# zblz/naima

Hardware: AMD Instinct MI355X
Metric: walker-steps/sec (ensemble lnprob evals/s) (higher is better)
Workload: dtype f64

## Files before the change

### naima_amd/csrc/nh_halfstep.hip

```cpp
#include "nh_hs_plan.h"
#include <memory>

typedef int hs_i16 __attribute__((ext_vector_type(16)));
typedef int hs_i8 __attribute__((ext_vector_type(8)));
typedef int hs_i2 __attribute__((ext_vector_type(2)));
typedef int hs_i4 __attribute__((ext_vector_type(4)));
template <class T>
__device__ __forceinline__ const T __attribute__((address_space(1))) * hs_gptr(int lo, int hi) {
  return (const T __attribute__((address_space(1)))*)(((unsigned long long)(unsigned)hi << 32) |
                                                      (unsigned)lo);
}
#define HS_KERNARG_H 48
static_assert(offsetof(hs_hot, F) == 0, "hs_first leads the argument block");
static_assert(sizeof(hs_hot) + HS_KERNARG_H <= 0xcc0, "the warm-up loads cover the argument block");
static_assert(sizeof(hs_hot) + HS_KERNARG_H >= 0xc84, "the last warm-up load (0xc80) stays inside the argument block");
static_assert(sizeof(hs_first) == 256 && offsetof(hs_first, qT) == 224 &&
                  offsetof(hs_first, syn_c) == 240 && offsetof(hs_first, nG) == 48 &&
                  offsetof(hs_first, e) == 64 && offsetof(hs_first, lne) == 128 &&
                  offsetof(hs_first, pkd) == 192, "hs_first: the layout the first trip reads");
__device__ __attribute__((noinline)) double hs_log_ool(double x) { return log(x); }
template <bool SYN, bool S2 = false>
__global__ __launch_bounds__(1024) void k_half_step(const int* __restrict__ done_,
                                                    const double* __restrict__ blk_,
                                                    const double* coords_, int slice, int ns_,
// ... 975 lines not shown
}

extern "C" int nh_table_interleave(nh_ctx* c, const double* Kt, const double* dlnKt,
                                   const double* lx, int nG, int nK, double* KD) {
  NH_REQUIRE(c && Kt && dlnKt && KD && nG >= 0 && nK >= 0, "bad argument");
  const long long n = (long long)nG * nK;
  if (n == 0) return NH_OK;
  nh_prof_scope ps(c, NH_K_TABLES);
  hipLaunchKernelGGL(k_table_interleave, dim3((unsigned)((n + 255) / 256)), dim3(256), 0, c->stream,
                     Kt, dlnKt, lx, nG, nK, KD);
  NH_CHECK_HIP(hipGetLastError());
  return NH_OK;
}

__global__ void k_syn_consts(const double* __restrict__ gam, const double* __restrict__ lx, int nG,
                             double* __restrict__ out) {
  const int i = blockIdx.x * blockDim.x + threadIdx.x;
  if (i >= nG) return;
  const double gi = gam[i];
  const double v = 1.0 / (gi * gi);
  out[i] = v;
  out[nG + i] = cbrt(v);
  out[2 * nG + i] = i + 1 < nG ? v * expm1(-2.0 * lx[i]) : 0.0;
}

__global__ void k_set_word(int* p, int v) { *p = v; }
__global__ void k_set_word2(int* p, int v0, int v1) {
  p[0] = v0;
  p[1] = v1;
}

__global__ void k_hist_append(const double* __restrict__ coords, const double* __restrict__ logp,
                              long long N, int ndim, const nh_hist* hist, long long row) {
  if (row < 0) row = hist->n - 1;
  if (!hist->coords || row < 0 || row >= hist->cap) return;
  const long long nc = N * ndim;
  double* hc = hist->coords + row * nc;
  double* hl = hist->logp + row * N;
  for (long long t = threadIdx.x; t < nc; t += blockDim.x) hc[t] = coords[t];
  for (long long t = threadIdx.x; t < N; t += blockDim.x) hl[t] = logp[t];
}

extern "C" int nh_hist_append(nh_ctx* c, const double* coords, const double* logp, long long N,
                              int ndim, const nh_hist* hist, long long row) {
  NH_REQUIRE(c && coords && logp && hist && N >= 1 && ndim >= 1, "bad argument");
  nh_prof_scope ps(c, NH_K_GLUE);
  hipLaunchKernelGGL(k_hist_append, dim3(1), dim3(1024), 0, c->stream, coords, logp, N, ndim, hist,
                     row);
  NH_CHECK_HIP(hipGetLastError());
  return NH_OK;
}

static hs_opt hs_env_opt(const char* name) {
  const char* e = getenv(name);
  hs_opt o;
  o.set = e != nullptr;
  o.v = e ? atoi(e) : 0;
  return o;
}
hs_knobs hs_knobs_read() {
  hs_knobs k = hs_knobs_default();
  k.test_reject = getenv("NH_HS_TEST_REJECT") != nullptr;
  if (const char* e = getenv("NH_HS_SPLIT")) k.kmax = atoi(e) > 0 ? atoi(e) : 1;
  k.part_kb = nh_env_int("NH_HS_PART_KB", k.part_kb);
  k.threads = hs_env_opt("NH_HS_THREADS");
  k.split_min_work = nh_env_int("NH_HS_SPLIT_MIN_WORK", k.split_min_work);
  k.rowsplit = nh_env_int("NH_HS_ROWSPLIT", k.rowsplit);
  k.rt = nh_env_int("NH_HS_RT", k.rt);
  k.syn2 = nh_env_int("NH_HS_SYN2", k.syn2);
  k.rt_debug = getenv("NH_HS_RT_DEBUG") != nullptr;
  k.seg = hs_env_opt("NH_HS_SEG");
  k.syn_nodes = hs_env_opt("NH_HS_SYN_NODES");
  k.debug = nh_env_int("NH_HS_DEBUG", 0) != 0;
  k.run_rt = nh_env_int("NH_RUN_RT", k.run_rt);
  k.run_grids_in_lds = nh_env_int("NH_RUN_GRIDS_IN_LDS", k.run_grids_in_lds);
  k.run_ut = nh_env_int("NH_RUN_UT", k.run_ut);
  k.run_rowsplit = nh_env_int("NH_RUN_ROWSPLIT", k.run_rowsplit);
  k.run_syn2 = nh_env_int("NH_RUN_SYN2", k.run_syn2);
  k.run_il = nh_env_int("NH_RUN_IL", k.run_il);
  k.run_rebalance = hs_env_opt("NH_RUN_REBALANCE");
  k.run_tcompact_min = nh_env_int("NH_RUN_TCOMPACT_MIN", k.run_tcompact_min);
  k.run_syn_nodes = hs_env_opt("NH_RUN_SYN_NODES");
  k.run_pipeline = nh_env_int("NH_RUN_PIPELINE", k.run_pipeline);
  k.run_fail_at = nh_env_int("NH_RUN_FAIL_AT", 0);
  k.run_grid = hs_env_opt("NH_RUN_GRID");
  k.run_max_per_wg = hs_env_opt("NH_RUN_MAX_PER_WG");
  k.run_shared_alloc = nh_env_int("NH_RUN_SHARED_ALLOC", k.run_shared_alloc);
  k.run_spin_limit = hs_env_opt("NH_RUN_SPIN_LIMIT");
  k.run_publish_delay = nh_env_int("NH_RUN_PUBLISH_DELAY", 0);
  return k;
}

bool hs_read_grid(const double* xg, int nG, std::vector<double>& out) {
  out.assign((size_t)nG, 0.0);
  if (hipMemcpy(out.data(), xg, (size_t)nG * sizeof(double), hipMemcpyDeviceToHost) == hipSuccess) return true;
  (void)hipGetLastError();
  return false;
}

static void hs_gather(nh_ctx* c, const nh_hs_desc* d, const hs_knobs& k, hs_facts& f, std::vector<double>& xg) {
  f.ncu = nh_cu_count(256);
  f.syn_xg = nullptr;
  for (int t = 0; t < HS_MAX_TAB; ++t) f.r0[t] = -1;
  if (d->ngrids < 1 || d->ngrids > NH_MAX_GRIDS) return;
  const bool want_xg = d->syn.grid >= 0 && d->syn.grid < d->ngrids && k.syn2 != 0 &&
                       d->grids[d->syn.grid].xg && d->grids[d->syn.grid].nG >= 2;
  const bool want_rows = hs_plan_reads_rows(d, k, f.ncu);
  if ((!want_xg && !want_rows) || nh_sync(c) != NH_OK) return;
  if (want_xg && hs_read_grid(d->grids[d->syn.grid].xg, d->grids[d->syn.grid].nG, xg)) f.syn_xg = xg.data();
  for (int t = 0; t < d->ntab && want_rows; ++t) {
    const nh_hs_table& tb = d->tab[t];
    if (tb.grid < 0 || tb.grid >= d->ngrids || !tb.KD || tb.nK < 1 || d->grids[tb.grid].nG < 2) break;
    const int nG = d->grids[tb.grid].nG, nK = tb.nK;
    if ((size_t)nG * nK * 16 > ((size_t)64 << 20)) break;
    std::vector<double> kd((size_t)nG * nK * 2);
    if (hipMemcpy(kd.data(), tb.KD, kd.size() * sizeof(double), hipMemcpyDeviceToHost) != hipSuccess) {
      (void)hipGetLastError();
      break;
    }
    int r0 = nG - 1;
    for (int i = 0; i < nG - 1 && r0 == nG - 1; ++i)
      for (int q = 0; q < nK; ++q)
        if (kd[((size_t)i * nK + q) * 2] != 0.0) { r0 = i; break; }
    f.r0[t] = r0;
  }
}

static int hs_create(nh_ctx* c, const nh_hs_desc* d, nh_halfstep_plan** out) {
  NH_REQUIRE(c && d && out, "NULL pointer");
  const hs_knobs k = hs_knobs_read();
  hs_facts facts;
  std::vector<double> xg;
  hs_gather(c, d, k, facts, xg);
  std::unique_ptr<nh_halfstep_plan> P(new nh_halfstep_plan());
  hs_hot& H = P->hot;
  hs_shape S;
  const int rc = hs_plan(d, k, facts, H, S);
  if (rc != NH_OK) return rc;
  P->span = 3;
  P->lds_bytes = S.lds_bytes;
  P->lds_core = S.lds_core;
  P->threads = S.threads;
  P->blocks = d->nloc;
  P->split = S.split;
  P->rowsplit = S.rowsplit ? 1 : 0;
  P->rt = S.rt ? 1 : 0;
  nh_owned& m = P->mem;
  const int nspec = H.C.nspec;
  if (k.debug) {
    P->dbg = m.dev<long long>(67840 * sizeof(long long));
    m.fill(c, P->dbg, 0, 67840 * sizeof(long long));
  }
  P->dev = m.dev<nh_pack>(sizeof(S.packs));
  if (H.syn_grid >= 0) {
    const int nGs = H.nG[H.syn_grid];
    const size_t ns2 = H.o_s2 ? HS_S2_HDR + S.s2.data.size() : 0;
    P->syn_c = m.dev<double>((3 * (size_t)nGs + ns2) * sizeof(double));
    if (m.ok()) {
      hipLaunchKernelGGL(k_syn_consts, dim3((unsigned)((nGs + 255) / 256)), dim3(256), 0, c->stream,
                         H.xg[H.syn_grid], H.lx[H.syn_grid], nGs, P->syn_c);
      m.check(hipGetLastError());
    }
    if (m.ok() && ns2) {
      const hs_s2_host& s2h = S.s2;
      std::vector<double> up(ns2, 0.0);
      up[0] = s2h.par.ilx; up[1] = s2h.par.th; up[2] = s2h.par.im; up[3] = s2h.par.lml;
// ... 162 lines not shown
```

### naima_amd/csrc/nh_hs_plan.h

```cpp
#pragma once
#include "nh_hs.h"
#include "nh_syn2.h"

#define HS_RUN_MAX_STEPS 32
#define HS_RUN_ERR_TIMEOUT 1
#define HS_RUN_ERR_PEER 2
#define HS_RUN_ERR_LAST_ROW 3
#define HS_RUN_MAX_RANKS 8
#define HS_RUN_HEAD 512
#define HS_O_HX 56
enum { HX_PRE = 0, HX_SPECRD = 1 };
#define HS_O_LNA 48
#define HS_RUN_TRAIL 16
#define HS_RUN_PKW 8

enum { HSU_FL = 0, HSU_NL, HSU_G, HSU_W, HSU_D, HSU_DP, HSU_IL, HSU_TH, HSU_LX, HSU_LNE, HSU_GX, HSU_GE,
       HSU_S2LW, HSU_S2LG, HSU_SC_LO, HSU_SC_HI, HSU_N };
static_assert(HSU_N == 16, "a unit's descriptor is four 16-byte reads");

enum { HST_KD_LO = 0, HST_KD_HI, HST_NK, HST_NG, HST_AW, HST_AD, HST_AL, HST_FLAGS, HST_SUB, HST_NKP,
       HST_N = 16 };
#define HSI_N 4

struct hs_run {
  unsigned long long* ring;
  int* status;
  int* accw;
  double* hcoords; double* hlogp;
  double* hblob[NH_HS_MAX_BLOB];
  long long hrow0, hcap;
  long long* dbg;
  double* xspec; int* tick;
  int slice0, nslices;
  unsigned seq;
  int gr, N;
  int o_gx[NH_MAX_GRIDS], o_lne[NH_MAX_GRIDS], o_ge[NH_MAX_GRIDS];
  int o_pk, o_small1, o_olds;
  int o_lcl;
  int o_trail;
  const double* kds[HS_MAX_TAB];
  int spin_limit;
  int syn_nodes;
  int rebalance;
  int* report;
  int report_launch;
  int* lcnt;
  int o_il[NH_MAX_GRIDS];
  int o_ut;
  int o_it;
  int o_sum, o_cmp;
  int o_pci;
  int o_mt;
  int o_lnt;
  int o_synce;
  int rowsplit;
  int tcompact;
  int o_rs;
  int nxmax;
  int sum_cols;
  int nrank, rank;
  unsigned long long* peer[HS_RUN_MAX_RANKS];
  int* nacc_own;
  int* hacc;
  int* curstamp;
  int stamp0;
  int publish_delay;
  int syn2, s2_own;
  int o_s2tab, o_s2lw, o_s2ig, o_s2lg, o_s2q, o_s2z, o_s2t;
  const double* s2_dev;
  hs_syn2_par s2;
  double s2_z0, s2_invd;
  double s2_r746;
  double s2_lnw0;
  int pipeline;
  long long* clk;
};

static_assert(sizeof(hs_hot) + sizeof(hs_run) <= 4000, "both argument blocks fit the kernarg segment");

struct hs_opt {
  bool set;
  int v;
  int or_else(int dflt) const { return set ? v : dflt; }
};
struct hs_knobs {
  bool test_reject;
  int kmax;
  int part_kb;
  hs_opt threads;
  int split_min_work;
  int rowsplit, rt, syn2;
  bool rt_debug;
  hs_opt seg, syn_nodes;
  bool debug;
  int run_rt, run_grids_in_lds, run_ut, run_rowsplit, run_syn2, run_il;
  hs_opt run_rebalance;
  int run_tcompact_min;
  hs_opt run_syn_nodes;
  int run_pipeline;
  int run_fail_at;
  hs_opt run_grid;
  hs_opt run_max_per_wg;
  int run_shared_alloc;
  hs_opt run_spin_limit;
  int run_publish_delay;
};
static inline hs_knobs hs_knobs_default() {
  hs_knobs k;
  memset(&k, 0, sizeof(k));
  k.kmax = 8; k.part_kb = 40; k.split_min_work = 1 << 20;
  k.rowsplit = k.rt = k.syn2 = 1;
  k.run_rt = k.run_grids_in_lds = k.run_ut = k.run_rowsplit = k.run_syn2 = k.run_il = 1;
  k.run_tcompact_min = 4; k.run_pipeline = 1; k.run_shared_alloc = 1;
  return k;
}

struct hs_facts {
  int ncu;
  const double* syn_xg;
  int r0[HS_MAX_TAB];
};
static inline bool hs_plan_reads_rows(const nh_hs_desc* d, const hs_knobs& k, int ncu) {
  return d->syn.grid < 0 && d->ntab > 0 && d->ntab <= NH_HS_MAX_TAB && d->nloc <= ncu && k.rt != 0;
}

#define HSP_REQUIRE(cond, msg)                                               \
  do {                                                                       \
    if (!(cond)) return nh_set_error(NH_EINVAL, "%s: %s", who, msg);         \
  } while (0)
#define HS_S2_HDR 16

struct hs_shape {
  int threads, split, segscale;
  bool rowsplit, rt;
  size_t lds_core, lds_bytes;
  hs_s2_host s2;
  nh_pack packs[NH_MAX_PACK];
};
struct hs_plan_front {
  int off, nspec, syn_nE, threads;
  long long work;
  bool s2_ok;
};

static inline int hs_plan_checked(const nh_hs_desc* d, const hs_knobs& k, const hs_facts& f, hs_hot& H,
                                  hs_shape& S, hs_plan_front& A) {
  static const char* who = "hs_create";
  HSP_REQUIRE(d->coords && d->logp && d->blk && d->cursor && d->qT && d->factors && d->params &&
                  d->total, "NULL pointer in the descriptor");
  HSP_REQUIRE(d->ns >= 1 && d->ndim >= 1 && d->ndim <= 64 && d->lo >= 0 && d->nloc >= 1 &&
                  d->lo + d->nloc <= d->ns, "bad proposal block");
  HSP_REQUIRE(!d->do_accept || (d->lo == 0 && d->nloc == d->ns && d->accepted),
              "the in-kernel accept needs every walker of the slice in this launch");
  HSP_REQUIRE(d->npacks >= 1 && d->npacks <= NH_MAX_PACK, "bad pack plan");
  HSP_REQUIRE(d->kind >= NH_PD_POWERLAW && d->kind <= NH_PD_LOGPARABOLA, "unknown particle distribution kind");
  HSP_REQUIRE(d->ngrids >= 1 && d->ngrids <= NH_MAX_GRIDS, "bad grid count");
  HSP_REQUIRE(d->nmoms >= 0 && d->nmoms <= NH_MAX_MOMENT, "bad reductions");
  HSP_REQUIRE(d->ntab >= 0 && d->ntab <= NH_HS_MAX_TAB && (d->ntab > 0 || d->syn.grid >= 0),
              "a half-step needs at least one emission component");
  HSP_REQUIRE(d->ncomp >= 1 && d->ncomp <= NH_MAX_COMP && d->nE >= 1, "bad likelihood components");
  HSP_REQUIRE(d->conv && d->flux && d->err_lo && d->err_hi && d->ul && d->cl, "NULL data column");
  HSP_REQUIRE(d->nterms >= 0 && d->nterms <= NH_MAX_PRIOR, "bad prior terms");
  static_assert(NH_HS_MAX_TAB == HS_MAX_TAB, "table count");
  static_assert(sizeof(hs_hot) <= 3800, "the by-value kernel argument must fit the 4 KB segment");
  memset(&H, 0, sizeof(H));
  hs_dev& C = H.C;
  memset(S.packs, 0, sizeof(S.packs));
  H.coords = d->coords; H.logp = d->logp; H.blk = d->blk; H.cursor = d->cursor;
  H.qT = d->qT; H.factors = d->factors; H.hist = d->hist;
  H.ns = d->ns; H.ndim = d->ndim; H.lo = d->lo; H.nloc = d->nloc;
  C.npk = d->npacks; C.kind = d->kind; C.params = d->params;
  bool have_params = false;
  for (int q = 0; q < d->npacks; ++q) {
    const nh_pack& pk = d->packs[q];
    HSP_REQUIRE(pk.out && pk.ncols >= 1 && pk.ncols <= NH_MAX_LAZY && pk.ld >= pk.ncols,
                "bad pack request");
    for (int c = 0; c < pk.ncols; ++c) {
      const double* b = pk.cols[c].base;
      HSP_REQUIRE(b == nullptr || (b >= d->qT && b < d->qT + (long long)d->ndim * d->nloc &&
                                   (b - d->qT) % d->nloc == 0 && pk.cols[c].stride == 1),
                  "a pack column must read one proposal coordinate (or be a constant)");
    }
    if (pk.out == d->params) {
      HSP_REQUIRE(pk.ncols >= 7, "the particle rows need 7 columns");
      have_params = true;
    }
    S.packs[q] = pk;
  }
  HSP_REQUIRE(have_params, "params must be the output of one of the packs");
  HSP_REQUIRE(d->ndim < 255, "at most 254 fit parameters");
  for (int t = 0; t < d->ntab; ++t) {
    const nh_hs_table& tb = d->tab[t];
    HSP_REQUIRE(tb.grid >= 0 && tb.grid < d->ngrids && tb.KD && tb.out && tb.nK >= 1 &&
                    tb.ldo >= tb.nK, "bad table reduction");
  }
  if (k.test_reject)
// ... 304 lines not shown
  bool rt = P->rt != 0 && H.syn_grid < 0 && H.ntab > 0 && P->threads <= 512 && k.run_rt != 0;
  rt = rt && H.C.nT <= (P->threads / 64) * P->split;
  const bool grids_in_lds = (P->threads >= 1024 || rt) && k.run_grids_in_lds != 0;
  for (int g = 0; g < NH_MAX_GRIDS; ++g) R.o_gx[g] = R.o_lne[g] = R.o_ge[g] = -1;
  for (int g = 0; g < H.ngrids && grids_in_lds; ++g) {
    R.o_gx[g] = off; off += H.nG[g];
    R.o_lne[g] = off; off += H.nG[g];
    R.o_ge[g] = off;
    if (H.F.broken & 1) off += H.nG[g];
  }
  for (int g = 0; g < NH_MAX_GRIDS; ++g) R.o_il[g] = -1;
  R.rebalance = k.run_rebalance.or_else(H.syn_grid < 0 ? 1 : 0);
  const bool units_tab = grids_in_lds && k.run_ut != 0;
  R.rowsplit = (P->rowsplit && P->split >= 2 && units_tab && R.rebalance && H.ntab == 1 &&
                HS_CHUNKS(H.C.tab[0].chunks) % P->split == 0 && H.C.nT % P->split == 0 &&
                k.run_rowsplit != 0) ? 1 : 0;
  R.tcompact = P->split >= k.run_tcompact_min ? 1 : 0;
  int hole_lo = 0, hole_hi = 0;
  if (R.tcompact) {
    int nsmax = 0;
    if (H.syn_grid >= 0) nsmax = (H.syn_nE * H.C.syn_cdmax + 63) / 64;
    const int nslots = R.rowsplit ? H.C.nT / P->split : (H.C.nT + nsmax) / P->split + 2;
    if (nslots < H.C.nT) {
      hole_lo = H.o_part_t + nslots * 64;
      hole_hi = H.o_part_t + H.C.nT * 64;
    } else {
      R.tcompact = 0;
    }
  }
  auto take = [&](int n, bool align16) {
    if (align16) hole_lo += hole_lo & 1;
    if (hole_lo + n <= hole_hi) {
      const int at = hole_lo;
      hole_lo += n;
      return at;
    }
    if (align16) off += off & 1;
    const int at = off;
    off += n;
    return at;
  };
  R.o_ut = -1;
  if (units_tab) {
    int nunits = 0;
    for (int g = 0; g < H.ngrids; ++g) nunits += (H.nG[g] + 63) / 64;
    R.o_ut = take(nunits * (HSU_N / 2), true);
  }
  {
    int ncols = 0;
    for (int t = 0; t < H.ntab; ++t) ncols += H.C.tab[t].nK;
    R.sum_cols = ncols;
    R.o_sum = take(ncols, false);
    R.o_cmp = take(2 * NH_MAX_COMP + 2, false);
    R.o_pci = take((NH_MAX_PRIOR + 1) / 2, false);
    R.o_synce = H.syn_grid >= 0 ? take(H.syn_nE, false) : -1;
    R.o_lnt = -1;
    R.o_mt = take(4 * NH_MAX_MOMENT, true);
    {
      int nun = 0;
      for (int g = 0; g < H.ngrids; ++g) nun += (H.nG[g] + 63) / 64;
      R.o_rs = take((9 + nun + 2 * NH_MAX_GRIDS + 1) / 2, false);
    }
    R.nxmax = H.C.nspec + NH_MAX_MOMENT;
  }
  for (int t = 0; t < H.ntab; ++t)
    HSP_REQUIRE(H.nG[H.C.tab[t].grid] < 65536, "a table's grid has too many nodes for the items' descriptors");
  R.o_it = -1;
  if (!rt && H.C.nT > 0)
    R.o_it = take((HS_MAX_TAB * HST_N + H.C.nT * HSI_N + 1) / 2, true);
  R.o_pk = take(NH_MAX_PACK * NH_MAX_LAZY * HS_RUN_PKW, false);
  R.o_small1 = take(HS_O_T64, false);
  R.o_olds = take(128, false);
  R.o_lcl = take(H.nE + 1, false);
  R.o_trail = take((HS_RUN_TRAIL * HS_MAX_TAB + H.C.nspec + 1) / 2, false);
  for (int t = 0; t < H.ntab; ++t)
    HSP_REQUIRE(H.C.tab[t].tiles <= HS_RUN_TRAIL, "a table of more column tiles than the resident loop stages");
  R.syn2 = 0;
  R.s2_dev = nullptr;
  if (H.syn_grid >= 0 && k.run_syn2 != 0 && syn_xg != nullptr &&
      hs_s2_prepare(syn_xg, H.nG[H.syn_grid], H.scale[H.syn_grid], 8, S.s2)) {
    const int nG = H.nG[H.syn_grid], Pn = S.s2.par.P;
    R.s2 = S.s2.par;
    R.s2_invd = S.s2.invd; R.s2_lnw0 = S.s2.lnw0; R.s2_z0 = S.s2.z0; R.s2_r746 = S.s2.r746;
    const int off_was = off, hole_was = hole_lo;
    R.o_s2tab = take((Pn + 1) * HS_S2_STRIDE, true);
    const int sg = H.syn_grid;
    bool own = nG >= 2 * HS_S2_GUARD && H.o_d[sg] == H.o_w[sg] + nG && H.o_ig23 == H.o_dig2 + nG;
    for (int t = 0; t < H.ntab; ++t) own = own && H.C.tab[t].grid != sg;
    for (int q = 0; q < H.nmom; ++q) own = own && H.mgrid[q] != sg;
    R.s2_own = own ? 1 : 0;
    if (own) {
      R.o_s2lw = H.o_w[sg];
      R.o_s2ig = H.o_dig2;
    } else {
      R.o_s2lw = take(nG + 2 * HS_S2_GUARD, false);
      R.o_s2ig = take(nG + 2 * HS_S2_GUARD, false);
    }
    if (own && grids_in_lds) {
      R.o_s2lg = R.o_gx[sg];
    } else {
      R.o_s2lg = take(nG, false);
    }
    R.o_s2q = take(4 * H.syn_nE, false);
    R.o_s2z = take((H.syn_nE + 1) / 2, false);
    R.o_s2t = take(HS_S2_TN, false);
    R.o_lnt = take(256, true);
    if ((size_t)off * sizeof(double) <= 160 * 1024) {
      R.syn2 = 1;
    } else {
      off = off_was;
      hole_lo = hole_was;
    }
  }
  if (k.run_il != 0)
    for (int g = 0; g < H.ngrids; ++g)
      if (H.o_dp[g] >= 0 && (hole_lo + H.nG[g] <= hole_hi || (size_t)(off + H.nG[g]) * sizeof(double) <= 158 * 1024))
        R.o_il[g] = take(H.nG[g], false);
  R.syn_nodes = H.C.syn_nodes;
  if (P->split == 1 && R.syn_nodes < 32) R.syn_nodes = R.syn2 ? 48 : 32;
  if (P->split == 2 && R.syn_nodes < 10) R.syn_nodes = 10;
  if (R.syn2 && P->split >= 2 && R.syn_nodes < 16) R.syn_nodes = 16;
  R.syn_nodes = k.run_syn_nodes.or_else(R.syn_nodes);
  R.pipeline = k.run_pipeline;
  if (k.run_fail_at > 0)
    fprintf(stderr, "libnaima_hip: NH_RUN_FAIL_AT=%d -- that launch of the resident loop is made to time "
                    "out (fault injection of the tests)\n", k.run_fail_at);
  HSP_REQUIRE(R.syn_nodes >= 1, "NH_RUN_SYN_NODES must be positive");
  const size_t lds = (size_t)off * sizeof(double);
  HSP_REQUIRE(lds <= 160 * 1024, "the resident loop's working set does not fit in LDS");
  S.rt = rt;
  S.lds_bytes = lds;
  return NH_OK;
}

static inline int hs_run_grid(const nh_halfstep_plan* P, bool shared, bool rt, const hs_run& R, const hs_knobs& k,
                              int per_cu, int ncu, int* grid, bool* deep_candidate) {
  static const char* who = "hs_run_create";
  const hs_hot& H = P->hot;
  HSP_REQUIRE(per_cu >= 1 && ncu >= 1, "the resident kernel does not fit a compute unit");
  long long cap = (long long)per_cu * ncu;
  if (k.run_grid.set) cap = k.run_grid.v > 0 ? k.run_grid.v : cap;
  const long long per_wg = k.run_max_per_wg.or_else(P->threads >= 1024 ? 8 : 1);
  HSP_REQUIRE((long long)H.nloc * P->split <= cap * (per_wg > 1 ? per_wg : 1),
              "more walkers per half-step than resident workgroups");
  *grid = (int)(H.nloc < cap / P->split ? H.nloc : cap / P->split);
  *deep_candidate = !shared && !rt && H.syn_grid >= 0 && P->split == 1 && P->threads >= 1024 &&
                    H.nloc > *grid && R.pipeline != 0;
  return NH_OK;
}

hs_knobs hs_knobs_read();
bool hs_read_grid(const double* xg, int nG, std::vector<double>& out);
```

### naima_amd/csrc/nh_persist.hip

```cpp
#include "nh_hs_plan.h"
#include <memory>
#include <vector>
#include <chrono>
#include <unistd.h>

#ifndef HS_RUN_PK
#define HS_RUN_PK 5
#endif

__device__ __forceinline__ unsigned long long hs_ld_sc1(const unsigned long long* p) {
  return __hip_atomic_load(p, __ATOMIC_RELAXED, __HIP_MEMORY_SCOPE_AGENT);
}
__device__ __forceinline__ void hs_st_sc1(unsigned long long* p, unsigned long long v) {
  __hip_atomic_store(p, v, __ATOMIC_RELAXED, __HIP_MEMORY_SCOPE_AGENT);
}
__device__ __forceinline__ unsigned long long hs_ld_sys(const unsigned long long* p) {
  return __hip_atomic_load(p, __ATOMIC_RELAXED, __HIP_MEMORY_SCOPE_SYSTEM);
}
__device__ __forceinline__ void hs_st_sys(unsigned long long* p, unsigned long long v) {
  __hip_atomic_store(p, v, __ATOMIC_RELAXED, __HIP_MEMORY_SCOPE_SYSTEM);
}
__device__ __forceinline__ unsigned hs_tag(unsigned seq, int row) {
  return (seq << 8) | (unsigned)(row + 1);
}
// ... 243 lines not shown
#define HSR_STAMP(k)                                                                   \
  do {                                                                                  \
    if (R.dbg && tid == 0 && blockIdx.x < 256 && it < 64)                               \
      R.dbg[((long long)blockIdx.x * 64 + it) * 8 + (k)] = (long long)wall_clock64();   \
  } while (0)

struct hsr_a_out { double pval; int pcol, bad, ok; };
template <bool SYN, bool MULTI, bool S2, int RT = 0, bool DEEP = false>
__global__ __launch_bounds__(RT > 0 ? 512 : 1024) void k_half_step_run(const hs_hot H, const hs_run R) {
  extern __shared__ double sm[];
  const hs_dev& D = H.C;
  const int T = blockDim.x, tid0 = threadIdx.x;
  const int wv = __builtin_amdgcn_readfirstlane(tid0 >> 6), nwv = T >> 6;
  int tid = tid0, lane = tid0 & 63;
  const int ns = H.ns, ndim = H.ndim, N = R.N;
  const int K = gridDim.y, part = blockIdx.y;
  const bool has_syn = SYN && H.syn_grid >= 0;
  const bool broken = (H.F.broken & 1) != 0;
  const int GRn = 2 * (ndim + 1);
  const bool lik_wave = wv == (nwv > 1 ? 1 : 0);
  const int npk8 = H.F.npk8;
  constexpr bool multi = MULTI;

  if (blockIdx.x == 0 && blockIdx.y == 0 && tid0 == 0) nh_clk_open(R.clk);
  if (wv == nwv - 1) sm[HS_O_T64 + lane] = exp2((double)lane * 0.015625);
  if (DEEP && tid0 < 2) {
    int* hx0 = reinterpret_cast<int*>((tid0 ? sm + R.o_small1 : sm) + HS_O_HX);
    hx0[HX_PRE] = 0;
    hx0[HX_SPECRD] = 0;
  }
  for (int g = 0; g < H.ngrids; ++g) {
    const int nG = H.nG[g];
    for (int i = tid; i < nG; i += T) {
      sm[H.o_lx[g] + i] = i + 1 < nG ? H.lx[g][i] : 0.0;
      if (R.o_il[g] >= 0) {
        const double il = i + 1 < nG ? nh_rcp(H.lx[g][i]) : 0.0;
        sm[R.o_il[g] + i] = il;
        sm[H.o_th[g] + i] = NH_SEG_SMALL_POS * il;
      }
      if (R.o_gx[0] >= 0) {
        if (!(SYN && S2 && R.s2_own && g == H.syn_grid)) sm[R.o_gx[g] + i] = H.xg[g][i];
        sm[R.o_lne[g] + i] = H.lne[g][i];
        if (broken) sm[R.o_ge[g] + i] = H.e[g][i];
      }
    }
  }
  {
    const int npri = (int)(sizeof(nh_prior_pack) / sizeof(double));
    const double* psrc = reinterpret_cast<const double*>(&D.pri);
    for (int t = tid; t < npri; t += T) sm[H.o_pri + t] = psrc[t];
    for (int t = tid; t < NH_MAX_PRIOR; t += T) {
      int ci = -1;
      if (t < D.pri.n && D.pri.t[t].x.base) {
        const long long d = D.pri.t[t].x.base - H.qT;
        if (d >= 0 && d < (long long)H.ndim * H.nloc && d % H.nloc == 0 && D.pri.t[t].x.stride == 1)
          ci = (int)(d / H.nloc);
      }
      reinterpret_cast<int*>(sm + R.o_pci)[t] = ci;
    }
    if (has_syn) {
      for (int k = tid; k < H.syn_nE; k += T) {
        const double E = H.syn_E[k];
        sm[H.o_synE + k] = E;
        sm[R.o_synce + k] = (1.7320508075688772 * (NH_E_GAUSS * NH_E_GAUSS * NH_E_GAUSS)) /
                            (2.0 * NH_PI * NH_M_E_G * (NH_C_CGS * NH_C_CGS) * NH_HBAR_CGS * (E * NH_ERG_PER_EV));
      }
      const int nGs = H.F.syn_nG;
      for (int i = tid; i < nGs; i += T) {
        sm[H.o_ig2 + i] = H.F.syn_c[i];
        if (!(S2 && R.s2_own)) {
          sm[H.o_ig23 + i] = H.F.syn_c[nGs + i];
          sm[H.o_dig2 + i] = H.F.syn_c[2 * nGs + i];
        }
      }
    }
    if (SYN && S2) {
      const int nGs = H.F.syn_nG, ntb = (R.s2.P + 1) * HS_S2_STRIDE;
      for (int i = tid; i < ntb; i += T) sm[R.o_s2tab + i] = R.s2_dev[i];
      for (int i = tid; i < HS_S2_TN; i += T) sm[R.o_s2t + i] = exp2((double)i * (1.0 / HS_S2_TN));
      if (tid < 128) {
        const double c = 0.5 + ((double)tid + 0.5) * (1.0 / 256.0);
        sm[R.o_lnt + 2 * tid] = 1.0 / c;
        sm[R.o_lnt + 2 * tid + 1] = log(c);
      }
      for (int i = tid; i < nGs; i += T) sm[R.o_s2lg + i] = R.s2_dev[ntb + i];
      for (int i = tid; i < nGs + 2 * HS_S2_GUARD; i += T) {
        const int ii = min(max(i - HS_S2_GUARD, 0), nGs - 1);
        sm[R.o_s2ig + i] = H.F.syn_c[ii];
        if (i < HS_S2_GUARD || i >= nGs + HS_S2_GUARD) sm[R.o_s2lw + i] = HS_S2_FLOOR;
      }
    }
    for (int t = 0; t < H.ntab; ++t)
      for (int k = tid; k < H.tnK[t]; k += T)
        sm[H.o_scale + H.tspec[t] + k] = H.tscale[t] ? H.tscale[t][k] : 1.0;
    double* lik = sm + H.o_lik;
    for (int k = tid; k <= H.nE; k += T) sm[R.o_lcl + k] = k < H.nE ? log(1.0 - H.cl[k]) : 0.0;
    for (int k = tid; k < H.nE; k += T) {
      lik[k] = H.conv[k];
      lik[H.nE + k] = H.flux[k];
      lik[2 * H.nE + k] = -0.5 / (H.elo[k] * H.elo[k]);
      lik[3 * H.nE + k] = -0.5 / (H.ehi[k] * H.ehi[k]);
      lik[4 * H.nE + k] = (double)H.ul[k];
    }
    int ko = H.o_mkt;
    for (int m = 0; m < H.nmom; ++m) {
      const int nG = H.nG[H.mgrid[m]];
      for (int i = tid; i < nG; i += T) {
        sm[ko + i] = H.mKt[m][i];
        sm[ko + nG + i] = H.mdK[m][i];
      }
      ko += 2 * nG;
    }
    {
      int* tr = reinterpret_cast<int*>(sm + R.o_trail);
      for (int t = 0; t < H.ntab; ++t) {
        const hs_tab& tb = D.tab[t];
        const double* kds = t == 0 ? R.kds[0] : t == 1 ? R.kds[1] : t == 2 ? R.kds[2] : R.kds[3];
        const bool has = kds != nullptr;
        const int* src = hs_tab_trailer(has ? kds : tb.KD, H.nG[tb.grid], tb.nK);
        for (int q = tid; q < HS_RUN_TRAIL; q += T) tr[t * HS_RUN_TRAIL + q] = has && q < HS_TRAIL_TILES ? src[q] : 0;
        for (int k = tid; k < tb.nK; k += T)
          tr[HS_RUN_TRAIL * HS_MAX_TAB + tb.spec_off + k] = has ? src[HS_TRAIL_TILES + k] : k;
      }
    }
    if (tid < npk8) {
      const nh_pack& P = D.pk[tid / NH_MAX_LAZY];
      const nh_lazy& z = P.cols[tid % NH_MAX_LAZY];
      double* o = sm + R.o_pk + tid * HS_RUN_PKW;
      o[6] = log(fabs(z.a));
      {
        const unsigned word = H.F.pkd[tid >> 2];
        const int b = (int)((word >> (8 * (tid & 3))) & 0xFFu);
        reinterpret_cast<int*>(o + 7)[0] = b != 0xFF ? b : -1;
        reinterpret_cast<int*>(o + 7)[1] = P.ncols > (int)(tid % NH_MAX_LAZY) ? 1 : 0;
      }
      o[0] = z.a;
      o[1] = z.b;
      o[2] = z.c;
      reinterpret_cast<int*>(o + 3)[0] = z.tf;
      reinterpret_cast<int*>(o + 3)[1] = P.ncols;
      reinterpret_cast<long long*>(o + 4)[0] = (long long)P.ld;
      reinterpret_cast<double**>(o + 5)[0] = P.out;
    }
  }
  if (R.o_ut >= 0) {
    int* ut = reinterpret_cast<int*>(sm + R.o_ut);
    int u0 = 0;
    for (int g = 0; g < H.ngrids; ++g) {
      const int nu = (H.nG[g] + 63) >> 6;
      const bool s2g = SYN && S2 && g == H.syn_grid;
      for (int q = tid; q < nu; q += T) {
        int* d = ut + (u0 + q) * HSU_N;
        const int i0 = q * 64;
        const bool dp = H.o_dp[g] >= 0, il = R.o_il[g] >= 0;
        auto at = [&](int off) { return (int)hs_lds_addr(sm + off + i0); };
        d[HSU_FL] = (s2g ? (R.s2_own ? 2 : 1) : 0) | (dp ? 4 : 0) | (dp && il ? 8 : 0);
        d[HSU_NL] = H.nG[g] - i0;
        d[HSU_G] = g;
        d[HSU_W] = at(H.o_w[g]);
        d[HSU_D] = at(H.o_d[g]);
        d[HSU_DP] = dp ? at(H.o_dp[g]) : 0;
        d[HSU_IL] = il ? at(R.o_il[g]) : 0;
        d[HSU_TH] = H.o_th[g] >= 0 ? at(H.o_th[g]) : 0;
        d[HSU_LX] = at(H.o_lx[g]);
        d[HSU_LNE] = at(R.o_lne[g]);
        d[HSU_GX] = at(R.o_gx[g]);
// ... 249 lines not shown
        double* qs = par_ ? sm + R.o_small1 : sm;
        double* row = qs + HS_O_ROW;
        double* lg = qs + HS_O_LG;
        double* accs = qs + HS_O_ACC;
        int* hi = reinterpret_cast<int*>(qs + HS_O_INT);
        int* hx = reinterpret_cast<int*>(qs + HS_O_HX);
        double* olds = sm + R.o_olds + par_ * 64;
        {
#define HSR_A_AHEAD true
#define HSR_A_NOT_YET return hsr_a_out{0.0, -1, 0, 0}
#include "nh_persist_phase_a.inc"
#undef HSR_A_AHEAD
#undef HSR_A_NOT_YET
        }
        {
#include "nh_persist_priors.inc"
        }
        return hsr_a_out{pval, pcol, slice_bad, 1};
      };
      bool pre_a = false;
      if constexpr (DEEP) pre_a = hx_cur[HX_PRE] != 0;
      const bool skip1 = pre_a;
      if (wv == 0 && !pre_a) {
        int* hx = hx_cur;
        (void)hx;
#define HSR_A_AHEAD false
#define HSR_A_NOT_YET do {} while (0)
#include "nh_persist_phase_a.inc"
#undef HSR_A_AHEAD
#undef HSR_A_NOT_YET
      }
      HSR_WSTAMP(0);
      if (!(DEEP && skip1)) __syncthreads();
      HSR_STAMP(2);
      if (RT == 0 && hi[HI_TICK] != 0) return;
      if (wv == 0 && pcol >= 0 && !slice_bad) {
        const double* o = sm + R.o_pk + lane * HS_RUN_PKW;
        const long long ld = reinterpret_cast<const long long*>(o + 4)[0];
        double* out = reinterpret_cast<double* const*>(o + 5)[0];
        out[(long long)j * ld + pcol] = pval;
      }
      HSR_FSTAMP(0);
      if (K > 1) {
        if (!R.tcompact)
          for (int t = tid; t < D.nT * 64; t += T) sm[H.o_part_t + t] = 0.0;
        if (has_syn)
          for (int t = tid; t < D.syn_cdmax * H.syn_nE; t += T) sm[H.o_part_s + t] = 0.0;
      }
      if (lik_wave && !(DEEP && pre_a)) {
#include "nh_persist_priors.inc"
      }
      const pd_par p = {row[0], row[1], row[2], row[3], row[4], row[5], row[6]};
      double* spec = sm + H.o_spec;
      double Bw = 0.0, qfac = 0.0;
      if (has_syn) Bw = D.syn_bcol >= 0 ? row[D.syn_bcol] : D.synB[(long long)j * D.syn_ldB];
      int lv_i0 = 0, lv_k = -1;
      double lv_q = 0.0, lv_E = 0.0;
      bool lv_live = false;
      int* tcnt = hi + 8;
      const int syn_tiles = tiles_;
      if (has_syn && nwv - 1 - wv < syn_tiles) {
        qfac = (NH_ERG_PER_EV * (2.0 * (NH_M_E_G * NH_C_CGS)) / (3.0 * NH_E_GAUSS * NH_HBAR_CGS)) * nh_rcp(Bw);
        const int nG = H.nG[H.syn_grid];
        const double* ig2 = sm + H.o_ig2;
        const int t = nwv - 1 - wv;
        lv_k = t * 64 + lane;
        lv_i0 = nG;
        double lv_lnq = 0.0;
        if (lv_k < H.syn_nE) {
          lv_E = sm[H.o_synE + lv_k];
          lv_q = lv_E * qfac;
          int lo = 0, hi2 = nG;
          if (S2) {
            lv_lnq = syn_tiles > 1 ? hsr_ln_tab(lv_q, hs_lds_addr(sm + R.o_lnt)) : hsr_log(lv_q);
            const double r = fma(lv_lnq, R.s2_invd, R.s2_r746);
            if (r == r) {
              int c = r > 0.0 ? (r < (double)nG ? (int)__builtin_ceil(r) : nG) : 0;
              const double xa = lv_q * ig2[max(c - 1, 0)], xb = lv_q * ig2[min(c, nG - 1)];
              if (!(c > 0 && c < nG && !(xa <= 746.0) && xb <= 746.0)) {
                while (c > 0 && lv_q * ig2[c - 1] <= 746.0) --c;
                while (c < nG && !(lv_q * ig2[c] <= 746.0)) ++c;
              }
              lo = c;
            } else {
              while (lo < hi2) {
                const int mid = (lo + hi2) >> 1;
                if (lv_q * ig2[mid] <= 746.0) hi2 = mid; else lo = mid + 1;
              }
            }
          } else {
            while (lo < hi2) {
              const int mid = (lo + hi2) >> 1;
              if (lv_q * ig2[mid] <= 746.0) hi2 = mid; else lo = mid + 1;
            }
          }
          lv_i0 = lo;
        }
        lv_live = lv_i0 < nG;
        const unsigned long long m = __builtin_amdgcn_ballot_w64(lv_live);
        int ln = lv_live ? (nG - 1) - lv_i0 : 0;
        ln = hs_wave_sum_i32_dpp(ln);
        if (lane == 63) {
          tcnt[t] = __popcll(m);
          if (ln > 0) atomicAdd(&hi[HI_LIVE], ln);
        }
        {
          const int nEs = H.syn_nE;
          int base = 0;
          for (int q = 0; q < t; ++q) {
            const int kq = q * 64 + lane;
            const bool lq = kq < nEs && (sm[H.o_synE + min(kq, nEs - 1)] * qfac) * ig2[nG - 1] <= 746.0;
            base += __popcll(__builtin_amdgcn_ballot_w64(lq));
          }
          int* amap = reinterpret_cast<int*>(sm + H.o_amap);
          int* ai0 = amap + nEs;
          double* sq = sm + H.o_sq;
          if (lv_live) {
            const int pos = base + __popcll(m & ((1ull << lane) - 1ull));
            amap[pos] = lv_k;
            ai0[pos] = lv_i0;
            const double cs1 = Bw * sm[R.o_synce + lv_k];
            if (!S2) {
              sq[pos] = lv_q;
              sq[nEs + pos] = hsr_cbrt(lv_q);
              sq[2 * nEs + pos] = cs1;
            }
            if (S2) {
              const double lnq = lv_lnq;
              const double z = fma(-lnq, R.s2_invd, R.s2_z0);
              const double Zf = floor(z);
              double* s2q = sm + R.o_s2q;
              s2q[pos] = lv_q;
              s2q[nEs + pos] = (HS_S2_LAMBDA / 3.0) * lnq;
              s2q[2 * nEs + pos] = (z - Zf) * R.s2.im;
              s2q[3 * nEs + pos] = cs1 * qs[HS_O_LNA + 1];
              reinterpret_cast<int*>(sm + R.o_s2z)[pos] = (int)Zf;
            }
          } else if (lv_k < nEs) {
            if (DEEP && skip1) {
              const int* hxp = reinterpret_cast<const int*>((par ? sm : sm + R.o_small1) + HS_O_HX);
              while (__atomic_load_n(&hxp[HX_SPECRD], __ATOMIC_RELAXED) == 0) __builtin_amdgcn_s_sleep(1);
              __builtin_amdgcn_fence(__ATOMIC_ACQUIRE, "workgroup");
            }
            spec[H.syn_spec_off + lv_k] = 0.0;
          }
        }
      }
      HSR_FSTAMP(1);
      if (R.o_ut >= 0) {
        const int* ul = reinterpret_cast<const int*>(sm + R.o_rs) + 9;
        const int u_end = R.rowsplit ? __builtin_amdgcn_readfirstlane(ul[-1]) : nunits;
        int fl = 0;
        for (int u = worker ? rank : u_end; u < u_end; u += 2 * nwork)
          fl |= hsr_weights_kind<(SYN && S2)>(
              D.kind, hs_lds_addr(sm + R.o_ut), R.rowsplit ? hs_lds_addr(reinterpret_cast<const double*>(ul)) : 0u,
              u, nwork, u_end, hs_lds_addr(row), hs_lds_addr(lg), hs_lds_addr(qs + HS_O_LNA),
              hs_lds_addr(sm + HS_O_T64), R.s2_lnw0);
        HSR_FSTAMP(4);
        fl = __builtin_amdgcn_readfirstlane(fl);
        if (lane == 0 && fl) atomicOr(&hi[HI_NZ], fl);
      } else {
      int nzmask = 0;
      for (int u = worker ? rank : nunits; u < nunits; u += 2 * nwork) {
        int gq[2], iq[2], bq[2] = {0, 0};
        double lrq[2] = {0.0, 0.0}, lneq[2] = {0.0, 0.0}, gxq[2] = {0.0, 0.0};
        bool onq[2];
// ... 1157 lines not shown
```

### naima_amd/csrc/nh_syn2.h

```cpp
#pragma once
#include "nh_common.h"

#define HS_S2_TTOP 7.0
#define HS_S2_TBOT (-46.0)
#define HS_S2_GUARD 16
#define HS_S2_TBITS 10
#define HS_S2_TN (1 << HS_S2_TBITS)
#define HS_S2_LAMBDA 1477.3197218702985
#define HS_S2_C 0.00067690154351557159L
#define HS_S2_FLOOR (-1.0e300)
#define HS_S2_DEG 5
#define HS_S2_STRIDE 6
#ifndef HS_S2_INLINE
#define HS_S2_INLINE __forceinline__
#endif

struct hs_syn2_par {
  int lm, P, nG, pad;
  double ilx, th, im, lml;
};

typedef double hs_s2_d2 __attribute__((ext_vector_type(2)));
typedef __attribute__((address_space(3))) const hs_s2_d2 hs_s2_lds_d2;
typedef __attribute__((address_space(3))) const double hs_s2_lds_d;
// ... 26 lines not shown
  const int k = (int)kf;
  unsigned j = (unsigned)(k & (HS_S2_TN - 1));
  asm("" : "+v"(j));
  return ldexp(hs_s2_ld(t128 + (j << 3)) * p, k >> HS_S2_TBITS);
}

__device__ __forceinline__ int hs_div_small(int x, int d, float rd) {
  int q = (int)((float)x * rd);
  const int r = x - q * d;
  q += r >= d ? 1 : 0;
  q -= r < 0 ? 1 : 0;
  return q;
}

__device__ HS_S2_INLINE void hs_syn2_item(int ix, int lane, int nA, int Cd, int nEs,
                                             const hs_syn2_par& S, const int* ai0, const int* Zs,
                                             const double* sq, unsigned a_lw, unsigned a_ig,
                                             unsigned a_tab, unsigned a_t128, double* part_s) {
  const int vt = ix * 64 + lane;
  const int ch = hs_div_small(vt, nA, __builtin_amdgcn_rcpf((float)nA));
  const int a = vt - ch * nA;
  if (ch >= Cd) return;
  const int lm = S.lm, m = 1 << lm;
  const int Z = Zs[a];
  const int k0 = ((Z + ai0[a]) >> lm) << lm;
  const int kend = Z + S.nG - 1;
  int per = hs_div_small(kend - k0 + Cd, Cd, __builtin_amdgcn_rcpf((float)Cd));
  per = ((per + m - 1) >> lm) << lm;
  const int kb = k0 + ch * per;
  double thE = 0x1p-10 * HS_S2_LAMBDA;
  asm volatile("" : "+s"(thE));
  double acc = 0.0;
  if (kb <= kend) {
    const int n = min(per, kend - kb + 1);
    const int groups = (n + m - 1) >> lm;
    const double qx = sq[a], Kc = sq[nEs + a], lam0 = sq[2 * nEs + a];
    double c0, c1, c2, c3, c4, c5;
    auto coefs = [&](int p, int kfirst, double& lam) {
      const int pe = min(p, S.P);
      const unsigned at = a_tab + (unsigned)pe * (8u * HS_S2_STRIDE);
      const hs_s2_d2 v01 = *(hs_s2_lds_d2*)(unsigned long long)at;
      const hs_s2_d2 v23 = *(hs_s2_lds_d2*)(unsigned long long)(at + 16u);
      const hs_s2_d2 v45 = *(hs_s2_lds_d2*)(unsigned long long)(at + 32u);
      c0 = v01.x + Kc; c1 = v01.y; c2 = v23.x; c3 = v23.y; c4 = v45.x; c5 = v45.y;
      lam = fma((double)(kfirst - (pe << lm)), S.im, lam0);
    };
    auto node = [&](unsigned pl, unsigned pg, double lam, double& E, double& u) {
      const double x = qx * hs_s2_ld(pg);
      double g = fma(c5, lam, c4);
      g = fma(g, lam, c3);
      g = fma(g, lam, c2);
      g = fma(g, lam, c1);
      g = fma(g, lam, c0);
      E = fma(x, -HS_S2_LAMBDA, g) + hs_s2_ld(pl);
      u = hs_exp128(E, a_t128);
    };
    double lam, E1, u1;
    coefs((kb >> lm) - 1, kb - m, lam);
    const int i0 = kb - 1 - Z;
    unsigned pl = a_lw + 8u * (unsigned)i0, pg = a_ig + 8u * (unsigned)i0;
    node(pl, pg, lam + S.lml, E1, u1);
    int kf = kb;
    for (int gi = 0; gi < groups; ++gi, kf += m) {
      coefs(kf >> lm, kf, lam);
      for (int j = 0; j < m; j += 2) {
        double EA, uA, EB, uB;
        node(pl + 8u, pg + 8u, lam, EA, uA);
        node(pl + 16u, pg + 16u, lam + S.im, EB, uB);
        acc = hs_seg_pre(acc, u1, uA, EA - E1, thE);
        acc = hs_seg_pre(acc, uA, uB, EB - EA, thE);
        E1 = EB;
        u1 = uB;
        lam += 2.0 * S.im;
        pl += 16u;
        pg += 16u;
      }
    }
  }
  double ilx_here = S.ilx;
  asm volatile("" : "+v"(ilx_here));
  part_s[ch * nEs + a] = acc * (sq[3 * nEs + a] * nh_rcp(ilx_here));
}

static inline long double hs_s2_rho(long double t) {
  const long double s = expl(2.0L * t / 3.0L);
  return logl((1.0L + 2.210L * s + 0.347L * s * s) /
              ((1.0L + 1.353L * s + 0.217L * s * s) * sqrtl(1.0L + 3.4L * s)));
}
static inline void hs_s2_piece(int p, long double h, double* c ) {
  const int n = HS_S2_DEG + 1;
  long double A[HS_S2_DEG + 1][HS_S2_DEG + 2];
  for (int r = 0; r < n; ++r) {
    const long double lam = 0.5L * (1.0L + cosl((2 * r + 1) * 3.14159265358979323846264L / (2 * n)));
    long double pw = 1.0L;
    for (int k = 0; k < n; ++k) { A[r][k] = pw; pw *= lam; }
    A[r][n] = (long double)HS_S2_LAMBDA * (hs_s2_rho((long double)HS_S2_TTOP - (p + lam) * h) + logl(1.808L));
  }
  for (int k = 0; k < n; ++k) {
    int piv = k;
    for (int r = k + 1; r < n; ++r) if (fabsl(A[r][k]) > fabsl(A[piv][k])) piv = r;
    for (int q = 0; q <= n; ++q) { const long double t = A[k][q]; A[k][q] = A[piv][q]; A[piv][q] = t; }
    for (int r = k + 1; r < n; ++r) {
      const long double f = A[r][k] / A[k][k];
      for (int q = k; q <= n; ++q) A[r][q] -= f * A[k][q];
    }
  }
  long double sol[HS_S2_DEG + 1];
  for (int k = n - 1; k >= 0; --k) {
    long double v = A[k][n];
    for (int q = k + 1; q < n; ++q) v -= A[k][q] * sol[q];
    sol[k] = v / A[k][k];
    c[k] = (double)sol[k];
  }
}

struct hs_s2_host {
  hs_syn2_par par;
  double invd, z0;
  double r746, lnw0;
  std::vector<double> data;
};
static inline bool hs_s2_prepare(const double* gam, int nG, double scale, int min_nodes, hs_s2_host& o) {
  bool ok = nG >= min_nodes && gam[0] > 0.0 && scale > 0.0;
  long double lx = 0.0L, dev = 0.0L;
  if (ok) {
    const long double l0 = logl((long double)gam[0]);
    lx = (logl((long double)gam[nG - 1]) - l0) / (nG - 1);
    for (int i = 0; i < nG && ok; ++i) {
      ok = gam[i] > 0.0;
      if (ok) dev = fmaxl(dev, fabsl(logl((long double)gam[i]) - l0 - i * lx));
    }
    ok = ok && lx > 0.0L && dev <= 1e-12L;
  }
  int lm = 0;
  if (ok) {
    lm = (int)lrint(log2(0.16 / (double)(2.0L * lx)));
    ok = lm >= 1 && lm <= 4;
  }
  if (!ok) return false;
  const int m = 1 << lm;
  const long double h = m * 2.0L * lx;
  const int P = (int)ceill(((long double)HS_S2_TTOP - (long double)HS_S2_TBOT) / h);
  o.data.assign((size_t)(P + 1) * HS_S2_STRIDE + nG, 0.0);
  for (int pc = 0; pc < P; ++pc) hs_s2_piece(pc, h, &o.data[(size_t)pc * HS_S2_STRIDE]);
  o.data[(size_t)P * HS_S2_STRIDE] = (double)((long double)HS_S2_LAMBDA * logl(1.808L));
  for (int i = 0; i < nG; ++i)
    o.data[(size_t)(P + 1) * HS_S2_STRIDE + i] =
        (double)((long double)HS_S2_LAMBDA * (logl((long double)gam[i]) / 3.0L + logl((long double)scale)));
  o.par.lm = lm; o.par.P = P; o.par.nG = nG; o.par.pad = 0;
  o.par.ilx = (double)(HS_S2_C / lx);
  o.par.th = (double)((long double)NH_SEG_SMALL_POS / lx);
  o.par.im = 1.0 / m;
  o.par.lml = (double)(m - 1) / m;
  o.invd = (double)(1.0L / (2.0L * lx));
  o.z0 = (double)(((long double)HS_S2_TTOP + 2.0L * logl((long double)gam[0])) / (2.0L * lx));
  o.lnw0 = (double)(-1075.0L * logl(2.0L) + logl((long double)NH_MEC2_EV / (long double)scale));
  o.r746 = (double)(((long double)HS_S2_TTOP - logl(746.0L)) / (2.0L * lx) -
                    ((long double)HS_S2_TTOP + 2.0L * logl((long double)gam[0])) / (2.0L * lx));
  return true;
}
```

Baseline: 13.49 million.

## Skip negligible synchrotron tail nodes using a provable per-walker cutoff bound

Adds a host-precomputed cutoff descriptor that lets the synchrotron inner loop start from a later grid node when a bound on the particle distribution's slope shows the skipped tail (x above ~128) contributes below f64 precision. The bound is checked per walker for each distribution kind, and the parameters are staged into LDS. This removes exp-heavy work on nodes whose contribution underflows, at the cost of extra per-row checks and a possible accuracy risk if the margin is wrong.

```diff
diff --git a/naima_amd/csrc/nh_halfstep.hip b/naima_amd/csrc/nh_halfstep.hip
--- a/naima_amd/csrc/nh_halfstep.hip
+++ b/naima_amd/csrc/nh_halfstep.hip
@@ -1081,6 +1081,7 @@
   k.run_tcompact_min = nh_env_int("NH_RUN_TCOMPACT_MIN", k.run_tcompact_min);
   k.run_syn_nodes = hs_env_opt("NH_RUN_SYN_NODES");
   k.run_pipeline = nh_env_int("NH_RUN_PIPELINE", k.run_pipeline);
+  k.run_syn_cut = nh_env_int("NH_RUN_SYN_CUT", k.run_syn_cut);
   k.run_fail_at = nh_env_int("NH_RUN_FAIL_AT", 0);
   k.run_grid = hs_env_opt("NH_RUN_GRID");
   k.run_max_per_wg = hs_env_opt("NH_RUN_MAX_PER_WG");
diff --git a/naima_amd/csrc/nh_hs_plan.h b/naima_amd/csrc/nh_hs_plan.h
--- a/naima_amd/csrc/nh_hs_plan.h
+++ b/naima_amd/csrc/nh_hs_plan.h
@@ -11,6 +11,7 @@
 #define HS_O_HX 56
 enum { HX_PRE = 0, HX_SPECRD = 1 };
 #define HS_O_LNA 48
+#define HS_O_S2CUT 32
 #define HS_RUN_TRAIL 16
 #define HS_RUN_PKW 8
 
@@ -72,6 +73,7 @@
   double s2_z0, s2_invd;
   double s2_r746;
   double s2_lnw0;
+  hs_s2_cut s2_cut;
   int pipeline;
   long long* clk;
 };
@@ -98,6 +100,7 @@
   int run_tcompact_min;
   hs_opt run_syn_nodes;
   int run_pipeline;
+  int run_syn_cut;
   int run_fail_at;
   hs_opt run_grid;
   hs_opt run_max_per_wg;
@@ -111,7 +114,7 @@
   k.kmax = 8; k.part_kb = 40; k.split_min_work = 1 << 20;
   k.rowsplit = k.rt = k.syn2 = 1;
   k.run_rt = k.run_grids_in_lds = k.run_ut = k.run_rowsplit = k.run_syn2 = k.run_il = 1;
-  k.run_tcompact_min = 4; k.run_pipeline = 1; k.run_shared_alloc = 1;
+  k.run_tcompact_min = 4; k.run_pipeline = 1; k.run_shared_alloc = 1; k.run_syn_cut = 1;
   return k;
 }
 
@@ -582,6 +585,8 @@
     const int nG = H.nG[H.syn_grid], Pn = S.s2.par.P;
     R.s2 = S.s2.par;
     R.s2_invd = S.s2.invd; R.s2_lnw0 = S.s2.lnw0; R.s2_z0 = S.s2.z0; R.s2_r746 = S.s2.r746;
+    R.s2_cut = S.s2.cut;
+    R.s2_cut.on = k.run_syn_cut != 0 ? 1 : 0;
     const int off_was = off, hole_was = hole_lo;
     R.o_s2tab = take((Pn + 1) * HS_S2_STRIDE, true);
     const int sg = H.syn_grid;
diff --git a/naima_amd/csrc/nh_persist.hip b/naima_amd/csrc/nh_persist.hip
--- a/naima_amd/csrc/nh_persist.hip
+++ b/naima_amd/csrc/nh_persist.hip
@@ -349,6 +349,13 @@
         const double c = 0.5 + ((double)tid + 0.5) * (1.0 / 256.0);
         sm[R.o_lnt + 2 * tid] = 1.0 / c;
         sm[R.o_lnt + 2 * tid + 1] = log(c);
+      }
+      if (tid == 0) {
+        double* cs = sm + HS_O_S2CUT;
+        cs[0] = R.s2_cut.rcut; cs[1] = R.s2_cut.span; cs[2] = R.s2_cut.lx; cs[3] = R.s2_cut.lne0m;
+        cs[4] = R.s2_cut.margin; cs[5] = R.s2_cut.lntcap;
+        reinterpret_cast<int*>(cs + 6)[0] = R.s2_cut.dref;
+        reinterpret_cast<int*>(cs + 6)[1] = R.s2_cut.on;
       }
       for (int i = tid; i < nGs; i += T) sm[R.o_s2lg + i] = R.s2_dev[ntb + i];
       for (int i = tid; i < nGs + 2 * HS_S2_GUARD; i += T) {
@@ -764,6 +771,23 @@
                 while (c < nG && !(lv_q * ig2[c] <= 746.0)) ++c;
               }
               lo = c;
+              const double* cs = sm + HS_O_S2CUT;
+              hs_s2_cut C;
+              C.rcut = cs[0]; C.span = cs[1]; C.lx = cs[2]; C.lne0m = cs[3]; C.margin = cs[4]; C.lntcap = cs[5];
+              C.dref = reinterpret_cast<const int*>(cs + 6)[0]; C.on = reinterpret_cast<const int*>(cs + 6)[1];
+              const int ic = hs_s2_cut_node(C, r, nG);
+              if (ic > c) {
+                const bool cut = hs_s2_cut_ok(C, D.kind, r, ic, nG, p.al, p.be, p.a2, lg[0], lg[1]);
+                if (cut) lo = ic;
+                if (R.dbg) {
+                  const int ncut = __popcll(__builtin_amdgcn_ballot_w64(cut));
+                  const int nkept = __popcll(__builtin_amdgcn_ballot_w64(!cut));
+                  if (lane == __builtin_ctzll(__builtin_amdgcn_ballot_w64(true))) {
+                    atomicAdd(reinterpret_cast<unsigned long long*>(R.dbg) + 256 * 64 * 8 + 11 * 16 + 0, (unsigned long long)ncut);
+                    atomicAdd(reinterpret_cast<unsigned long long*>(R.dbg) + 256 * 64 * 8 + 11 * 16 + 1, (unsigned long long)nkept);
+                  }
+                }
+              }
             } else {
               while (lo < hi2) {
                 const int mid = (lo + hi2) >> 1;
diff --git a/naima_amd/csrc/nh_syn2.h b/naima_amd/csrc/nh_syn2.h
--- a/naima_amd/csrc/nh_syn2.h
+++ b/naima_amd/csrc/nh_syn2.h
@@ -132,6 +132,52 @@
   part_s[ch * nEs + a] = acc * (sq[3 * nEs + a] * nh_rcp(ilx_here));
 }
 
+#define HS_S2_XCUT 128.0
+#define HS_S2_XREF 32.0
+#define HS_S2_TCAP 16.0
+struct hs_s2_cut {
+  double rcut;
+  double span;
+  double lx;
+  double lne0m;
+  double margin;
+  double lntcap;
+  int dref;
+  int on;
+};
+__host__ __device__ static inline int hs_s2_cut_node(const hs_s2_cut& C, double r, int nG) {
+  const double rc = r + C.rcut;
+  return rc > 0.0 ? (rc < (double)nG ? (int)ceil(rc) : nG) : 0;
+}
+__host__ __device__ static inline bool hs_s2_cut_ok(const hs_s2_cut& C, int kind, double r, int ic, int nG,
+                                                    double al, double be, double a2, double lg0, double lg1) {
+  if (!C.on || r != r || ic + C.dref + 1 > nG - 1) return false;
+  const double e_lo = fma(r, C.lx, C.lne0m), e_hi = fma(C.span, C.lx, e_lo);
+  double S, rem = C.margin;
+  bool ok = true;
+  switch (kind) {
+    case NH_PD_POWERLAW:
+    case NH_PD_ECPL:
+      S = al - 1.0;
+      break;
+    case NH_PD_BROKENPL:
+    case NH_PD_ECBPL:
+      S = (al > a2 ? al : a2) - 1.0;
+      ok = al == al && a2 == a2;
+      break;
+    default: {
+      const double s0 = fma(2.0 * be, e_lo - lg0, al - 1.0), s1 = fma(2.0 * be, e_hi - lg0, al - 1.0);
+      S = s0 > s1 ? s0 : s1;
+      ok = s0 == s0 && s1 == s1;
+    } break;
+  }
+  if (kind == NH_PD_ECPL || kind == NH_PD_ECBPL) {
+    ok = ok && be * ((be >= 0.0 ? e_hi : e_lo) - lg1) <= C.lntcap;
+    rem -= HS_S2_TCAP;
+  }
+  return ok && S == S && rem >= 0.0 && (S > 0.0 ? S : 0.0) * (C.span * C.lx) <= rem;
+}
+
 static inline long double hs_s2_rho(long double t) {
   const long double s = expl(2.0L * t / 3.0L);
   return logl((1.0L + 2.210L * s + 0.347L * s * s) /
@@ -168,8 +214,18 @@
   hs_syn2_par par;
   double invd, z0;
   double r746, lnw0;
+  hs_s2_cut cut;
   std::vector<double> data;
 };
+static inline long double hs_s2_g_extreme(long double t0, long double t1, int sign) {
+  long double best = -1e300L;
+  const int n = 4096;
+  for (int i = 0; i <= n; ++i) {
+    const long double t = t0 + (t1 - t0) * i / n;
+    best = fmaxl(best, sign * (t / 3.0L + logl(1.808L) + hs_s2_rho(t)));
+  }
+  return best;
+}
 static inline bool hs_s2_prepare(const double* gam, int nG, double scale, int min_nodes, hs_s2_host& o) {
   bool ok = nG >= min_nodes && gam[0] > 0.0 && scale > 0.0;
   long double lx = 0.0L, dev = 0.0L;
@@ -207,5 +263,20 @@
   o.lnw0 = (double)(-1075.0L * logl(2.0L) + logl((long double)NH_MEC2_EV / (long double)scale));
   o.r746 = (double)(((long double)HS_S2_TTOP - logl(746.0L)) / (2.0L * lx) -
                     ((long double)HS_S2_TTOP + 2.0L * logl((long double)gam[0])) / (2.0L * lx));
+  {
+    const long double d2 = 2.0L * lx, lc = logl((long double)HS_S2_XCUT), lr = logl((long double)HS_S2_XREF);
+    hs_s2_cut& c = o.cut;
+    c.rcut = (double)((logl(746.0L) - lc) / d2);
+    c.dref = (int)ceill((lc - lr) / d2) + 1;
+    c.span = c.rcut + c.dref + 3.0;
+    c.lx = (double)lx;
+    c.lne0m = (double)(logl((long double)gam[0]) + logl((long double)NH_MEC2_EV) - lx);
+    const long double gmax = hs_s2_g_extreme(lc - 1e-4L, logl(746.0L), 1);
+    const long double gmin = -hs_s2_g_extreme(lc - d2 * (c.dref + 2), lr, -1);
+    c.margin = (double)((long double)HS_S2_XCUT * (1.0L - 1e-4L) - (long double)HS_S2_XREF - (gmax - gmin) -
+                        60.0L * logl(2.0L) - logl((long double)nG) - 0.01L);
+    c.lntcap = log(HS_S2_TCAP);
+    c.on = 1;
+  }
   return true;
 }
```

Measured after the change: 13.74 million (median of 6 runs). 1.9% higher.
